# acoustic-warfare/beamforming-lk

Hardware: AMD Instinct MI355X
Metric: heatmap frames/sec (higher is better)
Workload: dtype f32

## Files before the change

### beamforming-lk_amd/_build.py

```python
from __future__ import annotations

import os
import shutil
import subprocess
from pathlib import Path

PKG_DIR = Path(__file__).resolve().parent
REPO = PKG_DIR.parent
CSRC = PKG_DIR / "csrc"
LIB_PATH = PKG_DIR / "libawpu_hip.so"

SOURCES = [CSRC / "das_kernels.hip", CSRC / "das_fast.hip", CSRC / "track_kernels.hip", CSRC / "block_kernels.hip", CSRC / "watch_kernels.hip", CSRC / "find_kernels.hip", CSRC / "band_kernels.hip", CSRC / "spectral_kernels.hip", CSRC / "expose_kernels.hip",
           CSRC / "awpu_hip.cpp", CSRC / "awpu_group.cpp", CSRC / "awpu_sweep.cpp", CSRC / "awpu_runs.cpp", CSRC / "geometry_host.cpp", CSRC / "find_host.cpp", CSRC / "band_host.cpp", CSRC / "spectral_host.cpp", CSRC / "awpu_focus.cpp", CSRC / "expose_host.cpp"]
GENERATOR = REPO / "tools" / "gen_trip_asm.py"
TRIP_INC = CSRC / "das_fast_trip.inc"
HEADERS = [CSRC / "awpu_handle.h", CSRC / "das_kernels.h", CSRC / "block_kernels.h", CSRC / "watch_kernels.h", CSRC / "find_kernels.h", CSRC / "find_rule.h", CSRC / "band_kernels.h", CSRC / "band_rule.h", CSRC / "spectral_kernels.h", CSRC / "spectral_rule.h", CSRC / "focus_rule.h", CSRC / "expose_kernels.h", CSRC / "expose_rule.h", CSRC / "nd_tile_window.h", CSRC / "sweep_plan.h", GENERATOR, REPO / "include" / "awpu_hip.h", REPO / "include" / "awpu_hip_track.h",
           REPO / "include" / "awpu_hip_blocks.h", REPO / "include" / "awpu_hip_listen.h", REPO / "include" / "awpu_hip_watch.h", REPO / "include" / "awpu_hip_find.h", REPO / "include" / "awpu_hip_band.h", REPO / "include" / "awpu_hip_focus.h", REPO / "include" / "awpu_hip_spectral.h", REPO / "include" / "awpu_hip_expose.h"]


def hipcc_path() -> str:
    for cand in (os.environ.get("HIPCC"), shutil.which("hipcc"), "/opt/rocm/bin/hipcc"):
        if cand and Path(cand).exists():
            return cand
    raise RuntimeError("hipcc not found: libawpu_hip.so cannot be built (there is no CPU fallback)")


def stale() -> bool:
    if not LIB_PATH.exists():
        return True
    built = LIB_PATH.stat().st_mtime
    return any(p.stat().st_mtime > built for p in SOURCES + HEADERS)


def build_library(force: bool = False, verbose: bool = False) -> Path:
    if not force and not stale():
        return LIB_PATH
    import fcntl

    with open(PKG_DIR / ".build.lock", "w") as lock:
        fcntl.flock(lock, fcntl.LOCK_EX)
        if not force and not stale():
            return LIB_PATH
        return _compile(verbose, force)


def generate_blocks(force: bool = False) -> Path:
    if not force and TRIP_INC.exists() and TRIP_INC.stat().st_mtime >= GENERATOR.stat().st_mtime:
        return TRIP_INC
    import sys
# ... 44 lines not shown
```

### beamforming-lk_amd/csrc/awpu_sweep.cpp

```cpp
#include "awpu_handle.h"

#include <algorithm>
#include <array>
#include <cstdio>
#include <cstdlib>
#include <cstring>
#include <map>
#include <vector>

#include "das_kernels.h"
#include "nd_tile_window.h"

using namespace awpu::host;

namespace {

int diag_begin(awpu_hip *h, size_t words, bool zero, hipStream_t s, unsigned long long **out) {
    if (const int rc = h->d_diag.ensure(words); rc != AWPU_OK) return rc;
    if (zero) AWPU_HIP_TRY(hipMemsetAsync(h->d_diag, 0, words * sizeof(unsigned long long), s));
    *out = h->d_diag;
    return AWPU_OK;
}

int diag_end(awpu_hip *h, int rc, size_t n_waves, int wg_waves, const char *tag, hipStream_t s) {
// ... 526 lines not shown
    a.n_pairs = (batch + 1) / 2;
    a.pair_group = awpu::xcd_pair_group((size_t) pp.usable_pad * pp.wr * 8, a.n_pairs);
    if (h->timing) AWPU_HIP_TRY(hipEventRecord(h->ev_begin, s));
    AWPU_HIP_TRY(awpu::launch_pack_pairs(d_frames, h->cfg.n_streams, hist_eff, wstart_eff, h->d_index, h->usable(), pp.usable_pad,
                                         h->d_gain, pp.wr, batch, h->d_pack, false, s));
    AWPU_HIP_TRY(awpu::launch_das_exact_quads(a, {table.entries, h->d_pack.cap}, s));
    return finish_launch(h, batch, s, AWPU_KERNEL_EXACT_QUAD);
}

int launch_exact_nd(awpu_hip *h, const float *d_frames, int batch, float *d_power, hipStream_t s, int hist_eff, int wstart_eff, int nq,
                    const float *prepacked = nullptr, size_t prepacked_floats = 0) {
    int rc = build_quad_lut(h, kQuadExactNd);
    if (rc != AWPU_OK) return rc;
    const QuadTable &table = h->quad_tables[kQuadExactNd];
    const awpu::FastPlan &pp = table.plan;
    if (!prepacked)
        if (const int prc = ensure_pack(h, pair_pack_floats(std::max(h->cfg.max_batch, batch), pp.usable_pad, pp.wr, 4)); prc != AWPU_OK) return prc;
    awpu::ExactNdArgs a{};
    fill_shared(a, h, pp, batch, d_power);
    a.packed = prepacked ? prepacked : h->d_pack;
    a.lut = table.d;
    a.sums = h->sums_out;
    a.wq = pp.wr;
    a.wq_tile = pp.row_bytes / 16;
    a.starts = h->d_nd_starts;
    a.start_entries = h->nd_start_entries;
    a.cols = h->cfg.grid_columns;
    a.rows = h->cfg.pixel_count / a.cols;
    a.nq = nq;
    a.tiles = awpu::nd_tiles(a.rows, a.cols, nq);
    a.n_pairs = (batch + 1) / 2;
    a.pair_group = awpu::xcd_pair_group((size_t) pp.usable_pad * pp.wr * 16, a.n_pairs, env().pair_group);
    if (env().pair_group <= 0 && a.pair_group == 2 && a.n_pairs >= 4 && (size_t) pp.usable_pad * pp.wr * 16 * 4 <= (6u << 20)) a.pair_group = 4;
    {
        const size_t items = (size_t) a.n_pairs * a.tiles;
        const long long key = ((long long) a.n_pairs << 24) | ((long long) a.pair_group << 8) | nq;
        if (!h->d_nd_items.holds(items)) {
            retire_live_graphs(h);
            AWPU_HIP_TRY(hipStreamSynchronize(s));
            if (rc = h->d_nd_items.grow(items); rc != AWPU_OK) return rc;
            h->nd_items_key = -1;
        }
        a.items = h->d_nd_items;
        a.build_items = h->nd_items_key != key;
        h->nd_items_key = key;
    }
    if (rc = arm_item_queues(h, a.n_pairs * a.tiles, &a.queue, &a.wgs, &a.tail); rc != AWPU_OK) return rc;
#ifdef AWPU_TUNING_BUILD
    if (const char *v = std::getenv("AWPU_ND_TAIL")) {
        const int per = (a.n_pairs * a.tiles + 7) / 8;
        a.tail = std::max(1, std::atoi(v) >= 100 ? per : per * std::atoi(v) / 100);
    }
#endif
    if (h->timing) AWPU_HIP_TRY(hipEventRecord(h->ev_begin, s));
    if (!prepacked) {
        AWPU_HIP_TRY(awpu::launch_pack_nd(d_frames, h->cfg.n_streams, hist_eff, wstart_eff, h->d_index, h->usable(), pp.usable_pad, h->d_gain,
                                          pp.wr, batch, h->d_pack, a.queue, s));
        a.queue_zeroed = 1;
    }
#ifdef AWPU_TUNING_BUILD
    const size_t n_wgs = std::min<size_t>((size_t) a.n_pairs * a.tiles, (size_t) a.wgs);
    if (env().debug & 16)
        if (const int drc = diag_begin(h, n_wgs * 8, true, s, &a.debug_out); drc != AWPU_OK) return drc;
#endif
    AWPU_HIP_TRY(awpu::launch_das_exact_nd(a, {table.entries, prepacked ? prepacked_floats : h->d_pack.cap}, s));
    rc = finish_launch(h, batch, s, AWPU_KERNEL_EXACT_ND);
#ifdef AWPU_TUNING_BUILD
    if (rc == AWPU_OK && (env().debug & 16)) return dump_nd_timeline(h, n_wgs, s);
#endif
    return rc;
}

bool takes_exact_nd(awpu_hip *h, int batch, int *nq) {
    if (!h->exact_pairs_ok || !h->exact_nd_ok || h->cfg.grid_columns < 1) return false;
    const ExactShape ex = env().exact_pairs;
    if (ex == ExactShape::kVerify || ex == ExactShape::kPair || ex == ExactShape::kQuad) return false;
    const int cols = h->cfg.grid_columns, rows = h->cfg.pixel_count / cols;
    const bool quads_pay = h->cfg.pixel_count % cols == 0 && h->cfg.pixel_begin % cols == 0 && h->quad_differ < 1.5;
    if ((!(h->pair_cols > 0 || quads_pay) && !forces_exact_nd(ex)) || rows < 4) return false;
    const long wgs2 = (long) awpu::nd_tiles(rows, cols, 2) * ((batch + 1) / 2);
    *nq = ex == ExactShape::kNd1 ? 1 : ex == ExactShape::kNd2 ? 2 : (rows >= 8 && wgs2 >= 512 ? 2 : 1);
    return true;
}

int arm_done_flag(awpu_hip *h, unsigned long long workgroups, awpu::DoneFlag *out) {
    if (!h->d_done_counter) {
        if (const int rc = h->d_done_counter.grow(1); rc != AWPU_OK) return rc;
        AWPU_HIP_TRY(hipMemsetAsync(h->d_done_counter, 0, sizeof(unsigned long long), h->stream));
        AWPU_HIP_TRY(hipStreamSynchronize(h->stream));
        if (const int rc = h->h_done_flag.grow(16); rc != AWPU_OK) return rc;
        *h->h_done_flag = 0;
        h->done_total = 0;
    }
    out->counter = h->d_done_counter;
    out->flag = h->h_done_flag;
    out->target = h->done_total + workgroups;
    out->seq = h->done_seq + 1;
    return AWPU_OK;
// ... 463 lines not shown
```

### beamforming-lk_amd/csrc/das_fast.hip

```cpp
#include "das_kernels.h"

#include <algorithm>
#include <atomic>

namespace awpu {

typedef float f2 __attribute__((ext_vector_type(2)));
typedef float f4 __attribute__((ext_vector_type(4)));
typedef float f4u __attribute__((ext_vector_type(4), aligned(4)));
typedef float f8 __attribute__((ext_vector_type(8)));

#define AWPU_AS4 __attribute__((address_space(4)))

typedef int i16 __attribute__((ext_vector_type(16)));

struct EntryGroup {
    i16 v;
    __device__ __forceinline__ float f(int k) const { return __int_as_float(v[4 * k + 0]); }
    __device__ __forceinline__ unsigned addr(int k) const { return (unsigned) v[4 * k + 1]; }
    __device__ __forceinline__ float g(int k) const { return __int_as_float(v[4 * k + 2]); }
};

template <int FPI>
struct Reads {
    f2 x[FPI], y[FPI];
};

__device__ __forceinline__ void no_fuse() { asm volatile("" ::: "memory"); }

template <int FPI>
__device__ __forceinline__ void issue_reads(Reads<FPI> &r, unsigned entry_addr, const char *lane_base) {
    constexpr int FS = kFastLdsBytes / FPI;
    const char *p = lane_base + entry_addr;
// ... 1072 lines not shown
    }
}

__device__ __forceinline__ f2 next_and_difference(float cur, float next, float gm) {
#pragma clang fp contract(off)
    const float c = cur * gm, n = next * gm;
    return f2{n, c - n};
}

__global__ void pack_nd_kernel(const float *frames, int n_streams, int hist, int wstart, const int32_t *index, int usable,
                               const float *gain, int wq, int batch, float *packed, unsigned *queue) {
    const int pair = blockIdx.y, s = blockIdx.x, rows_out = gridDim.x;
    if (queue && pair == 0 && s == 0 && threadIdx.x < 9) queue[threadIdx.x] = 0u;
    f4 *dst = (f4 *) packed + ((size_t) pair * rows_out + s) * wq;
    if (s >= usable) {
        for (int t = threadIdx.x; t < wq; t += blockDim.x) dst[t] = f4{0.0f, 0.0f, 0.0f, 0.0f};
        return;
    }
    const int fa = min(2 * pair, batch - 1), fb = min(2 * pair + 1, batch - 1);
    const float *xa = frames + ((size_t) fa * n_streams + index[s]) * hist + wstart;
    const float *xb = frames + ((size_t) fb * n_streams + index[s]) * hist + wstart;
    const float gm = gain ? gain[s] : 1.0f;
    const int valid = min(wq, hist - wstart - 1);
    for (int t = threadIdx.x; t < wq; t += blockDim.x) {
        f4 v = f4{0.0f, 0.0f, 0.0f, 0.0f};
        if (t < valid) {
            const f2 ea = next_and_difference(xa[t], xa[t + 1], gm), eb = next_and_difference(xb[t], xb[t + 1], gm);
            v = f4{ea.x, eb.x, ea.y, eb.y};
        }
        dst[t] = v;
    }
}

__global__ void nd_items_kernel(int2 *items, int n_pairs, int tiles, int pair_group, int tiles_per_row, int nq) {
    const int item = blockIdx.x * blockDim.x + threadIdx.x;
    if (item >= n_pairs * tiles) return;
    const int full_items = (n_pairs / pair_group) * pair_group * tiles;
    const int ga = item < full_items ? pair_group : n_pairs % pair_group;
    const int rem = item < full_items ? item : item - full_items;
    const int grp = rem / (tiles * ga), in = rem - grp * tiles * ga;
    const int tile = in / ga;
    const int pair = (item < full_items ? grp * pair_group : n_pairs - ga) + (in - tile * ga);
    const int rowq = tile / tiles_per_row, colt = tile - rowq * tiles_per_row;
    items[item] = int2{pair, (nq * rowq * tiles_per_row + colt) * 16};
}

struct NdQueues {
    unsigned *q;
    int per, total, tail;
    __device__ __forceinline__ int len(int x) const { return max(0, min(per, total - x * per)); }
    __device__ __forceinline__ int head(int x) const { return len(x) - min(len(x), tail); }
    __device__ __forceinline__ int take_head(int x) const {
        if (head(x) <= 0) return -1;
        const unsigned i = atomicAdd(&q[x], 1u);
        return i < (unsigned) head(x) ? x * per + (int) i : -1;
    }
    __device__ __forceinline__ int take_common() const {
        if (tail <= 0) return -1;
        for (;;) {
            const unsigned j = atomicAdd(&q[8], 1u);
            const int run = (int) (j / (unsigned) tail), k = (int) (j - (unsigned) run * (unsigned) tail);
            if (run >= 8) return -1;
            if (k < len(run) - head(run)) return run * per + head(run) + k;
        }
    }
    __device__ __forceinline__ int take(int xcd) const {
        int item = take_head(xcd);
        if (item < 0) item = take_common();
        for (int y = 1; item < 0 && y < 8; y++) item = take_head((xcd + y) & 7);
        return item;
    }
};

template <int NQ, bool SUMS>
__global__ __launch_bounds__(1024, 4) void das_exact_nd_kernel(ExactNdArgs a) {
    extern __shared__ __attribute__((aligned(16))) float lds[];
    constexpr int NW = 16, BUF = kFastLdsBytes;
    const int wave = __builtin_amdgcn_readfirstlane(threadIdx.x >> 6);
    const unsigned lds_base = (unsigned) (unsigned long long) (const __attribute__((address_space(3))) char *) lds;
    int *mail = (int *) (lds + 2 * (BUF / 4));
    const int total = a.n_pairs * a.tiles;
    unsigned xcc;
    asm volatile("s_getreg_b32 %0, hwreg(HW_REG_XCC_ID)" : "=s"(xcc));
    const NdQueues Q{a.queue, (total + 7) >> 3, total, a.tail};
    const int xcd = (int) (xcc & 7u);
    if (threadIdx.x == 0) {
        const int first = Q.take(xcd);
        mail[0] = first;
        mail[1] = first >= 0 ? Q.take(xcd) : -1;
    }
    __syncthreads();
    int cur = __builtin_amdgcn_readfirstlane(mail[0]), nxt = __builtin_amdgcn_readfirstlane(mail[1]);
    if (cur < 0) return;
    __syncthreads();

    const int tiles_per_row = (a.cols + NW - 1) / NW;
    auto decode = [&](int item, int &pair, int &tile_quad, const unsigned *&starts) {
        const int2 d = a.items[item];
        pair = __builtin_amdgcn_readfirstlane(d.x);
        tile_quad = __builtin_amdgcn_readfirstlane(d.y);
        const int quad_row = (tile_quad >> 4) / tiles_per_row, col_tile = (tile_quad >> 4) - quad_row * tiles_per_row;
        starts = a.starts + (size_t) ((quad_row >> 1) * tiles_per_row + col_tile) * a.usable_pad;
    };
    const int groups_total = a.usable_pad >> 2;
    const size_t row_floats = (size_t) a.wq * 4;
    const int n_chunks = (a.usable_pad + a.chunk - 1) / a.chunk;
    const int first_mics = min(a.chunk, a.usable_pad), last_mics = a.usable_pad - (n_chunks - 1) * a.chunk;
    const unsigned dbf = __builtin_amdgcn_readfirstlane((unsigned) ((size_t) a.chunk * row_floats * 4));
    const int row_bytes = a.wq_tile * 16;
    const int row_pieces = (row_bytes + 1023) >> 10;
    const unsigned last_shift = (unsigned) (row_pieces * 64 - a.wq_tile);
    const int rank = wave >> 2;
    const unsigned pka = __builtin_amdgcn_readfirstlane((unsigned) (first_mics >> 2) | (unsigned) (last_mics >> 2) << 8 | (unsigned) n_chunks << 16);
    const unsigned pkb_item = (wave < a.chunk ? (unsigned) row_pieces : 0u) | (wave < last_mics ? (unsigned) row_pieces : 0u) << 8 | last_shift << 24 |
                              (unsigned) rank << 30;
    const unsigned pkb_next = wave < first_mics ? (unsigned) row_pieces << 16 : 0u;
    const int own_head = Q.head(xcd);

    int pair, tile;
    const unsigned *starts;
    decode(cur, pair, tile, starts);
#ifdef AWPU_TUNING_BUILD
    const unsigned long long rt_begin = a.debug_out ? __builtin_amdgcn_s_memrealtime() : 0ull;
    long long t_sweep = 0, t_other = 0, t_mark = __builtin_readcyclecounter();
    int n_items = 0;
#endif
    {
        if (wave < first_mics) {
            const unsigned start = __builtin_amdgcn_readfirstlane(starts[wave]);
            const float *src = a.packed + ((size_t) pair * a.usable_pad + wave) * row_floats + (start >> 2);
            const int lane = (int) (threadIdx.x & 63);
            for (int k = 0; k < row_pieces; k++) {
                const int el = k * 64 + lane;
                if (el < a.wq_tile) {
                    float *dst = lds + ((wave * row_bytes) >> 2) + k * 256;
                    __builtin_amdgcn_global_load_lds((const __attribute__((address_space(1))) void *) (src + (size_t) el * 4),
                                                     (__attribute__((address_space(3))) void *) dst, 16, 0, 0);
                }
            }
        }
    }
    asm volatile("s_waitcnt vmcnt(0)" ::: "memory");
    __syncthreads();
    unsigned step = 0;

    for (;;) {
        const int cols_pad = tiles_per_row * NW;
        const int rowq = tile / (NQ * cols_pad);
        const int col = tile - NQ * rowq * cols_pad + wave;
        const int quad0 = tile + wave;
        const QuadEntry *quad_lut = a.lut + (size_t) quad0 * groups_total * 16;
        const float *pair_base = a.packed + (size_t) pair * a.usable_pad * row_floats;
        int pair_next = pair, tile_next = tile;
        const unsigned *starts_next = starts;
        if (nxt >= 0) decode(nxt, pair_next, tile_next, starts_next);
        const float *next_base = a.packed + (size_t) pair_next * a.usable_pad * row_floats;
        unsigned ticket = 0;
        const bool asked = wave == 0 && nxt >= 0 && own_head > 0;
        const unsigned *qptr = (const unsigned *) uniform_ptr(asked ? a.queue + xcd : nullptr);

        f8 O[NQ][4];
#ifdef AWPU_TUNING_BUILD
        { const long long n = __builtin_readcyclecounter(); t_other += n - t_mark; t_mark = n; }
#endif
        {
            unsigned tid = threadIdx.x;
            asm volatile("" : "+v"(tid));
            const unsigned lane_bytes = (tid & 63) * 16;
            const int buf = (int) (step & 1);
            unsigned lane_addr = lds_base + buf * BUF + lane_bytes;
            const unsigned ddst = __builtin_amdgcn_readfirstlane(lds_base + (buf ^ 1) * BUF + wave * row_bytes);
            const int delta = __builtin_amdgcn_readfirstlane(buf ? -BUF : BUF);
            const unsigned pkb = __builtin_amdgcn_readfirstlane(pkb_item | (nxt >= 0 ? pkb_next : 0u));
            const float *row_src = pair_base + (size_t) wave * row_floats, *row_next = next_base + (size_t) wave * row_floats;
            if constexpr (NQ == 1) {
                sweep_exact_nd_item1(O[0][0], O[0][1], O[0][2], O[0][3], uniform_ptr(quad_lut), pka, lane_addr, pkb, uniform_ptr(row_src), dbf,
                                     uniform_ptr(row_next), ddst, delta, lane_bytes, uniform_ptr(starts + wave), uniform_ptr(starts_next + wave), qptr, ticket);
            } else {
                static_assert(NQ == 2, "blocks are generated for one and two quads per wave");
                const int qstride = __builtin_amdgcn_readfirstlane(tiles_per_row * NW * groups_total * 16 * (int) sizeof(QuadEntry));
                sweep_exact_nd_item2(O[0][0], O[0][1], O[0][2], O[0][3], O[1][0], O[1][1], O[1][2], O[1][3], uniform_ptr(quad_lut), qstride, pka, lane_addr,
                                     pkb, uniform_ptr(row_src), dbf, uniform_ptr(row_next), ddst, delta, lane_bytes, uniform_ptr(starts + wave),
                                     uniform_ptr(starts_next + wave), qptr, ticket);
            }
            step += n_chunks;
        }
        if (threadIdx.x == 0 && nxt >= 0) {
            int got = own_head > 0 && ticket < (unsigned) own_head ? xcd * Q.per + (int) ticket : -1;
            if (got < 0) {
                got = Q.take_common();
                for (int y = 1; got < 0 && y < 8; y++) got = Q.take_head((xcd + y) & 7);
            }
            mail[0] = got;
        }
#ifdef AWPU_TUNING_BUILD
        { const long long n = __builtin_readcyclecounter(); t_sweep += n - t_mark; t_mark = n; n_items++; }
#endif

        unsigned tid_e = threadIdx.x;
        asm volatile("" : "+v"(tid_e));
        const int lane = (int) (tid_e & 63);
        const float norm = (float) (kSamples * a.usable);
#pragma unroll
        for (int q = 0; q < NQ; q++) {
            const int row4 = NQ * rowq + q;
            auto finish = [&](const f8 &Op, int pp) {
                const int row = 4 * row4 + pp;
                const bool live = row < a.rows && col < a.cols;
                const int p = min(row, a.rows - 1) * a.cols + min(col, a.cols - 1);
                f2 o[4];
#pragma unroll
                for (int k = 0; k < 4; k++) o[k] = f2{Op[2 * k], Op[2 * k + 1]};
                if (SUMS && live) {
#pragma unroll
                    for (int k = 0; k < 4; k++) {
                        a.sums[((size_t) (2 * pair) * a.pixel_count + p) * kSamples + lane + 64 * k] = o[k].x;
                        if (2 * pair + 1 < a.batch) a.sums[((size_t) (2 * pair + 1) * a.pixel_count + p) * kSamples + lane + 64 * k] = o[k].y;
                    }
                }
                return pixel_pair_partial_exact(o, lane);
            };
            const f2 s0 = finish(O[q][0], 0), s1 = finish(O[q][1], 1), s2 = finish(O[q][2], 2), s3 = finish(O[q][3], 3);
            const float sum = wave_sum8(s0.x, s0.y, s1.x, s1.y, s2.x, s2.y, s3.x, s3.y, lane);
            const int value = kWaveSum8Value(lane >> 3), row = 4 * row4 + (value >> 1), frame = 2 * pair + (value & 1);
            if ((lane & 7) == 0 && row < a.rows && col < a.cols && frame < a.batch)
                a.power[(size_t) frame * a.pixel_count + (size_t) row * a.cols + col] = sum / norm;
        }

        if (nxt < 0) break;
        __syncthreads();
        cur = nxt;
        pair = pair_next;
        tile = tile_next;
        starts = starts_next;
        nxt = __builtin_amdgcn_readfirstlane(mail[0]);
        __syncthreads();
    }
#ifdef AWPU_TUNING_BUILD
    if (a.debug_out && threadIdx.x == 0) {
        unsigned hw_id;
        asm volatile("s_getreg_b32 %0, hwreg(HW_REG_HW_ID)" : "=s"(hw_id));
        unsigned long long *o = a.debug_out + 8 * (size_t) blockIdx.x;
        o[0] = rt_begin;
        o[1] = __builtin_amdgcn_s_memrealtime();
        o[2] = (unsigned long long) t_other;
        o[3] = (unsigned long long) t_sweep;
        o[4] = (unsigned long long) (__builtin_readcyclecounter() - t_mark);
        o[5] = ((unsigned long long) xcc << 32) | hw_id;
        o[6] = (unsigned long long) n_items;
        o[7] = 1;
    }
#endif
}

__device__ __forceinline__ void store_tile_and_signal(float *lds, bool holder, int tile_row, int wave, int lane, float value, float *power, int row0,
                                                      int col0, int rows, int cols, const DoneFlag &done) {
    __syncthreads();
    if (holder) lds[tile_row * 16 + wave] = value;
    __syncthreads();
    if (wave != 0) return;
    const int r = row0 + (lane >> 4), c = col0 + (lane & 15);
    if (r < rows && c < cols) __hip_atomic_store(&power[(size_t) r * cols + c], lds[lane], __ATOMIC_RELAXED, __HIP_MEMORY_SCOPE_SYSTEM);
    asm volatile("s_waitcnt vmcnt(0)" ::: "memory");
    if (lane == 0 && __hip_atomic_fetch_add(done.counter, 1ull, __ATOMIC_RELAXED, __HIP_MEMORY_SCOPE_AGENT) + 1ull == done.target)
        __hip_atomic_store(done.flag, done.seq, __ATOMIC_RELAXED, __HIP_MEMORY_SCOPE_SYSTEM);
}

__global__ void pack_ndh_kernel(const float *frames, int n_streams, int pitch, int wstart, const int32_t *index, int usable,
// ... 349 lines not shown
        }
        sum.x = wave_sum(sum.x);
        sum.y = wave_sum(sum.y);
        const int p = pix[pp];
        if (lane == 0 && live[pp]) {
            a.power[(size_t) (2 * pair) * a.pixel_count + p] = sum.x / norm;
            if (2 * pair + 1 < a.batch) a.power[(size_t) (2 * pair + 1) * a.pixel_count + p] = sum.y / norm;
        }
    }
}

template <bool DIAG, int VAR>
__global__ __launch_bounds__(1024, 4) void das_quad_kernel(QuadArgs a) {
    extern __shared__ __attribute__((aligned(16))) float lds[];
    constexpr int NW = 16, kThreads = NW * 64, BUF = kFastLdsBytes;
    constexpr int kPieces = (BUF + kThreads * 16 - 1) / (kThreads * 16);
    const int lane = threadIdx.x & 63;
    const int wave = __builtin_amdgcn_readfirstlane(threadIdx.x >> 6);
    const unsigned lds_base = (unsigned) (unsigned long long) (const __attribute__((address_space(3))) char *) lds;

    const int total = a.n_pairs * a.tiles;
    const int per_xcd = (total + 7) >> 3;
    const int wgs_per_xcd = gridDim.x >> 3;
    const int run_begin = (blockIdx.x & 7) * per_xcd, run_end = min(total, run_begin + per_xcd);
    const int full_items = (a.n_pairs / a.pair_group) * a.pair_group * a.tiles;
    auto decode = [&](int item, int &pair, int &tile) {
        const int ga = item < full_items ? a.pair_group : a.n_pairs % a.pair_group;
        const int rem = item < full_items ? item : item - full_items;
        const int grp = rem / (a.tiles * ga), in = rem - grp * a.tiles * ga;
        tile = in / ga;
        pair = (item < full_items ? grp * a.pair_group : a.n_pairs - ga) + (in - tile * ga);
    };
    const bool queued = !DIAG && VAR == 0 && a.queue != nullptr;
    const NdQueues Q{a.queue, per_xcd, total, a.tail};
    int *mail = (int *) (lds + 2 * (BUF / 4));
    int xcd = (int) (blockIdx.x & 7);
    int item, nxt = -1;
    if (queued) {
        unsigned xcc;
        asm volatile("s_getreg_b32 %0, hwreg(HW_REG_XCC_ID)" : "=s"(xcc));
        xcd = (int) (xcc & 7u);
        if (threadIdx.x == 0) {
            const int first = Q.take(xcd);
            mail[0] = first;
            mail[1] = first >= 0 ? Q.take(xcd) : -1;
        }
        __syncthreads();
        item = __builtin_amdgcn_readfirstlane(mail[0]);
        nxt = __builtin_amdgcn_readfirstlane(mail[1]);
        if (item < 0) return;
        __syncthreads();
    } else {
        item = run_begin + (blockIdx.x >> 3);
        if (item >= run_end) return;
    }

    const int tiles_per_row4 = (a.cols + NW - 1) / NW;
    const int groups_total = a.usable_pad >> 2;
    const size_t row_floats = (size_t) a.wp * 2;
    const int n_chunks = (a.usable + a.chunk - 1) / a.chunk;
    const int rank = wave >> 2;
    const float norm = (float) (kSamples * a.usable);
    const int out_value = kWaveSum8Value(lane >> 3), out_pp = out_value >> 1, out_frame = out_value & 1;
    auto chunk_mics = [&](int m0) { return (min(a.chunk, a.usable - m0) + 3) & ~3; };
    const unsigned lane_bytes = threadIdx.x * 16;
    auto dma_chunk = [&](const float *src, int mc4, int buf) {
        const unsigned n_bytes = (unsigned) ((size_t) mc4 * row_floats * 4);
#pragma unroll
        for (int k = 0; k < kPieces; k++) {
            if (lane_bytes + k * kThreads * 16 < n_bytes) {
                const char *base = (const char *) uniform_ptr((const char *) src + k * kThreads * 16);
                float *dst = lds + buf * (BUF / 4) + (wave * 64 + k * kThreads) * 4;
                __builtin_amdgcn_global_load_lds((const __attribute__((address_space(1))) void *) (base + lane_bytes),
                                                 (__attribute__((address_space(3))) void *) dst, 16, 0, 0);
            }
        }
    };

// ... 19 lines not shown
    for (;;) {
        const int row4 = tile / tiles_per_row4;
        const int col = (tile - row4 * tiles_per_row4) * NW + wave;
        const int quad = row4 * tiles_per_row4 * NW + col;
        const QuadEntry *quad_lut = a.lut + (size_t) quad * groups_total * 16;
        const float *pair_base = a.packed + (size_t) pair * a.usable_pad * row_floats;
        const int item_next = queued ? nxt : item + wgs_per_xcd;
        const bool more = queued ? nxt >= 0 : item_next < run_end;
        int pair_next = 0, tile_next = 0;
        if (more) decode(item_next, pair_next, tile_next);

        f8 A0 = {0, 0, 0, 0, 0, 0, 0, 0}, A1 = A0, A2 = A0, A3 = A0, T = A0, V0 = A0, V2 = A0, V3 = A0;
        if constexpr (!DIAG && VAR == 0) {
            const int buf = step & 1;
            unsigned lane_addr = lds_base + buf * BUF + lane * 8;
            const int ngf = __builtin_amdgcn_readfirstlane(chunk_mics(0) >> 2);
            const int ngl = __builtin_amdgcn_readfirstlane(chunk_mics((n_chunks - 1) * a.chunk) >> 2);
            const unsigned dbf = __builtin_amdgcn_readfirstlane((unsigned) ((size_t) a.chunk * row_floats * 4));
            const unsigned dbl = __builtin_amdgcn_readfirstlane((unsigned) ((size_t) ngl * 4 * row_floats * 4));
            const float *nsrc = more ? a.packed + (size_t) pair_next * a.usable_pad * row_floats : pair_base;
            const unsigned dbn = __builtin_amdgcn_readfirstlane(more ? (unsigned) ((size_t) chunk_mics(0) * row_floats * 4) : 0u);
            const unsigned ddst = __builtin_amdgcn_readfirstlane(lds_base + (buf ^ 1) * BUF + wave * 1024);
            const int delta = __builtin_amdgcn_readfirstlane(buf ? -BUF : BUF);
            unsigned ticket = 0;
            const bool asked = queued && wave == 0 && more && Q.head(xcd) > 0;
            const unsigned *qptr = (const unsigned *) uniform_ptr(asked ? a.queue + xcd : nullptr);
            sweep_quad_item(A0, A1, A2, A3, T, V0, V2, V3, uniform_ptr(quad_lut), ngf, ngl, __builtin_amdgcn_readfirstlane(n_chunks),
                            lane_addr, rank, uniform_ptr(pair_base), dbf, dbl, uniform_ptr(nsrc), dbn, ddst, delta, lane_bytes, qptr, ticket);
            step += n_chunks;
            if (queued && threadIdx.x == 0 && more) {
                int got = Q.head(xcd) > 0 && ticket < (unsigned) Q.head(xcd) ? xcd * Q.per + (int) ticket : -1;
                if (got < 0) {
                    got = Q.take_common();
                    for (int y = 1; got < 0 && y < 8; y++) got = Q.take_head((xcd + y) & 7);
                }
                mail[0] = got;
            }
        } else
        for (int c = 0; c < n_chunks; c++, step++) {
            const int m0 = c * a.chunk;
            const int mc4 = chunk_mics(m0);
            const int buf = step & 1;
            long long t = DIAG ? __builtin_readcyclecounter() : 0;
            const int ng = __builtin_amdgcn_readfirstlane(mc4 >> 2);
            const int g_head = (a.debug & 512) ? __builtin_amdgcn_readfirstlane((ng * rank) >> 2) : 0;
            const unsigned lane_addr = lds_base + buf * BUF + lane * 8;
            auto sweep = [&](int g0, int n) {
                const void *row = uniform_ptr(quad_lut + (size_t) ((m0 >> 2) + g0) * 16);
                if constexpr (DIAG) {
                    unsigned dw = 0, da = 0;
                    sweep_quad_sum_stamped(A0, A1, A2, A3, T, V0, V2, V3, row, n, lane_addr, rank, dw, da);
                    t_wait += dw;
                    t_all += da;
                    n_blocks++;
                } else {
#ifdef AWPU_QUAD_VARIANTS
                    if constexpr (VAR == 1) sweep_quad_sum_v0(A0, A1, A2, A3, T, V0, V2, V3, row, n, lane_addr, rank);
                    else if constexpr (VAR == 2) sweep_quad_sum_v3(A0, A1, A2, A3, T, V0, V2, V3, row, n, lane_addr, rank);
                    else if constexpr (VAR == 3) sweep_quad_sum_v4(A0, A1, A2, A3, T, V0, V2, V3, row, n, lane_addr, rank);
                    else
#endif
                    sweep_quad_sum(A0, A1, A2, A3, T, V0, V2, V3, row, n, lane_addr, rank);
                }
            };
            const float *next_src = nullptr;
            int next_mc4 = 0;
            if (c + 1 < n_chunks) {
// ... 425 lines not shown
    if (a.cols > 0 && (unsigned) a.wp * 2u != kFirStaticPlaneBytes) return hipErrorInvalidValue;
    if ((a.wp & 3) || a.pair_group < 1 ||
        !within({(size_t) a.pixel_count * a.usable_pad + kFir8PlaneTablePrefetch, (size_t) n_pairs * a.usable * a.wp * 2}, have))
        return hipErrorInvalidValue;
    return launch_lds<das_fir8_plane_kernel<VAR>>(xcd_grid((long) n_pairs * n_tiles), dim3(1024), kTwoImages, stream, a,
                                                  (const FirPlaneEntry *) d_entries, d_coeffs, n_tiles, a.pair_group);
}

hipError_t launch_das_fir8_planes(const PairArgs &a, const void *d_entries, const float *d_coeffs, int variant, const Extents &have,
                                  hipStream_t stream) {
#ifdef AWPU_QUAD_VARIANTS
    if (variant == 1) return launch_fir8_plane_variant<1>(a, d_entries, d_coeffs, have, stream);
    if (variant == 2) return launch_fir8_plane_variant<2>(a, d_entries, d_coeffs, have, stream);
    if (variant == 3) return launch_fir8_plane_variant<3>(a, d_entries, d_coeffs, have, stream);
#endif
    (void) variant;
    return launch_fir8_plane_variant<0>(a, d_entries, d_coeffs, have, stream);
}

hipError_t launch_pack_nd(const float *d_frames, int n_streams, int hist, int wstart, const int32_t *d_index, int usable, int rows_out,
                          const float *d_gain, int wq, int batch, float *d_packed, unsigned *d_queue, hipStream_t stream) {
    hipLaunchKernelGGL(pack_nd_kernel, dim3(rows_out, (batch + 1) / 2), dim3(128), 0, stream, d_frames, n_streams, hist, wstart, d_index,
                       usable, d_gain, wq, batch, d_packed, d_queue);
    return hipGetLastError();
}

template <int NQ, bool SUMS>
static hipError_t launch_exact_nd_variant(const ExactNdArgs &a, hipStream_t stream) {
    const long total = (long) a.n_pairs * a.tiles;
    if (!a.queue_zeroed)
        if (hipError_t e = hipMemsetAsync(a.queue, 0, 9 * sizeof(unsigned), stream); e != hipSuccess) return e;
    if (a.build_items)
        hipLaunchKernelGGL(nd_items_kernel, dim3((unsigned) ((total + 255) / 256)), dim3(256), 0, stream, const_cast<int2 *>(a.items), a.n_pairs,
                           a.tiles, a.pair_group, (a.cols + 15) / 16, NQ);
    return launch_lds<das_exact_nd_kernel<NQ, SUMS>>(dim3((unsigned) std::min<long>(total, std::max(1, a.wgs))), dim3(1024),
                                                     kTwoImages + 64, stream, a);
}

hipError_t launch_das_exact_nd(const ExactNdArgs &a, const Extents &have, hipStream_t stream) {
    if ((a.nq != 1 && a.nq != 2) || !a.queue || !a.items || a.wgs < 1 || a.tail < 1) return hipErrorInvalidValue;
    if (!chunk_fits(a.chunk, a.usable_pad, (size_t) a.wq_tile * 16) || a.chunk > 16 || a.usable < 1 || a.usable > a.usable_pad || a.wq_tile < kSamples ||
        a.wq_tile > a.wq || !grid_is(a.rows, a.cols, a.pixel_count))
        return hipErrorInvalidValue;
    if (!items_agree(a.n_pairs, a.batch, a.tiles, nd_tiles(a.rows, a.cols, a.nq), a.pair_group)) return hipErrorInvalidValue;
    if (!a.starts || a.start_entries < (size_t) nd_tiles(a.rows, a.cols, 2) * a.usable_pad + 16) return hipErrorInvalidValue;
    if (!within({(size_t) nd_quad_count(a.rows, a.cols, a.nq) * (a.usable_pad / 4) * 16 + kQuadTablePrefetch,
                 (size_t) a.n_pairs * a.usable_pad * a.wq * 4}, have))
        return hipErrorInvalidValue;
    if (a.sums) return a.nq == 2 ? launch_exact_nd_variant<2, true>(a, stream) : launch_exact_nd_variant<1, true>(a, stream);
    return a.nq == 2 ? launch_exact_nd_variant<2, false>(a, stream) : launch_exact_nd_variant<1, false>(a, stream);
}

hipError_t launch_pack_ndh(const float *d_frames, int n_streams, int pitch, int wstart, const int32_t *d_index, int usable, int rows_out,
                           const float *d_gain, int wh, int batch, float *d_packed, hipStream_t stream) {
    hipLaunchKernelGGL(pack_ndh_kernel, dim3(rows_out, batch), dim3(256), 0, stream, d_frames, n_streams, pitch, wstart, d_index, usable, d_gain,
                       wh, d_packed);
    return hipGetLastError();
}

static bool ndh_shape_ok(const ExactNdhArgs &a, int tiles_of_grid, size_t image_bytes) {
    return chunk_fits(a.chunk, a.usable_pad, (size_t) a.wh * 16, image_bytes) && a.usable >= 1 && a.usable <= a.usable_pad && a.wh >= kSamples / 2 &&
           grid_is(a.rows, a.cols, a.pixel_count) && a.batch >= 1 && a.tiles == tiles_of_grid && (long) a.batch * a.tiles <= 0x7fffffffL;
}

template <int NQ, bool STATIONARY>
static hipError_t launch_exact_ndh_variant(const ExactNdhArgs &a, hipStream_t stream) {
    return launch_lds<das_exact_ndh_kernel<NQ, STATIONARY>>(dim3((unsigned) ((long) a.batch * a.tiles)), dim3(1024), kTwoImages, stream, a);
}

hipError_t launch_das_exact_ndh(const ExactNdhArgs &a, bool stationary, const Extents &have, hipStream_t stream) {
    if (a.nq != 1 && a.nq != 2) return hipErrorInvalidValue;
    if (!ndh_shape_ok(a, ndh_tiles(a.rows, a.cols, a.nq), stationary ? kTwoImages : kFastLdsBytes)) return hipErrorInvalidValue;
    if (stationary ? (a.chunk != a.usable_pad || !a.frames || !a.index || a.pitch < 1) : !a.packed) return hipErrorInvalidValue;
// ... 149 lines not shown
```

### beamforming-lk_amd/csrc/das_kernels.h

```cpp
#pragma once

#include <hip/hip_runtime.h>
#include <stdint.h>

#if defined(AWPU_TIMING_BUILD) && !defined(AWPU_TUNING_BUILD)
#define AWPU_TUNING_BUILD 1
#endif
#include "sweep_plan.h"

namespace awpu {

constexpr int kDebugNoRefill = 1, kDebugNoSweep = 2, kDebugNoTail = 4, kDebugNoBarrier = 8, kDebugRegStaging = 64;
constexpr int kDebugSafeBits = 16 | 256 | 512 | 4096;
#ifdef AWPU_TIMING_BUILD
#define AWPU_DBG(a, bit) ((a).debug & (bit))
#else
#define AWPU_DBG(a, bit) 0
#endif

struct LutEntry {
    int32_t off_rel;
    float frac;
};

// ... 68 lines not shown
    float *power;
    float *sums;
    int32_t usable, usable_pad, pixel_count, wp, chunk, batch;
    int32_t cols;
    int32_t tiles, n_pairs, pair_group;
};
hipError_t launch_das_exact_pairs(const ExactPairArgs &a, const Extents &have, hipStream_t stream);
struct ExactQuadArgs {
    const float *packed;
    const struct QuadEntry *lut;
    float *power;
    float *sums;
    int32_t usable, usable_pad, pixel_count, wp, chunk, batch;
    int32_t cols, rows;
    int32_t tiles, n_pairs, pair_group;
};
hipError_t launch_das_exact_quads(const ExactQuadArgs &a, const Extents &have, hipStream_t stream);
struct ExactNdArgs {
    const float *packed;
    const struct QuadEntry *lut;
    const unsigned *starts;
    size_t start_entries;
    int32_t wq_tile;
    float *power;
    float *sums;
    int32_t usable, usable_pad, pixel_count, wq, chunk, batch;
    int32_t cols, rows;
    int32_t nq;
    int32_t tiles, n_pairs, pair_group;
    unsigned *queue;
    int32_t queue_zeroed;
    int32_t wgs;
    int32_t tail;
    const int2 *items;
    int32_t build_items;
    unsigned long long *debug_out;
};
inline int nd_tiles(int rows, int cols, int nq) { return (((rows + 3) / 4 + nq - 1) / nq) * ((cols + 15) / 16); }
inline int nd_quad_count(int rows, int cols, int nq) { return (((rows + 3) / 4 + nq - 1) / nq) * nq * ((cols + 15) / 16) * 16; }
hipError_t launch_pack_nd(const float *d_frames, int n_streams, int hist, int wstart, const int32_t *d_index, int usable, int rows_out,
                          const float *d_gain, int wq, int batch, float *d_packed, unsigned *d_queue, hipStream_t stream);
hipError_t launch_das_exact_nd(const ExactNdArgs &a, const Extents &have, hipStream_t stream);
struct DoneFlag {
    unsigned long long *counter;
    unsigned *flag;
    unsigned long long target;
    uint32_t seq;
};
struct ExactNdhArgs {
    const float *packed;
    const float *frames;
    const struct QuadEntry *lut;
    const int32_t *index;
    const float *gain;
    float *power;
    float *sums;
    int32_t n_streams, pitch, wstart;
    int32_t usable, usable_pad, pixel_count, wh, chunk, batch;
    int32_t cols, rows;
    int32_t nq;
    int32_t tiles;
    int32_t lut_cols;
    int32_t identity;
    DoneFlag done;
};
inline int ndh_tiles(int rows, int cols, int nq) { return ((rows + 3) / 4) * ((cols + 16 * nq - 1) / (16 * nq)); }
// ... 210 lines not shown
```

Measured before the change: 24150.

## Claim runs of consecutive work items per queue ticket in exact ND kernel

Adds run-based work claiming to the exact ND kernel's per-XCD queues, so one atomic ticket can hand a workgroup up to four consecutive items. It also adds a tile_block ordering option to the item-list builder. The item descriptors for a run are prefetched through scalar loads, and the per-item block barriers and mailbox traffic are skipped inside a run. Both knobs default to 1 and can only be changed through environment variables in tuning builds, so the default path behaves like single-item claiming with some extra control flow.

```diff
diff --git a/beamforming-lk_amd/_build.py b/beamforming-lk_amd/_build.py
--- a/beamforming-lk_amd/_build.py
+++ b/beamforming-lk_amd/_build.py
@@ -14,7 +14,7 @@
            CSRC / "awpu_hip.cpp", CSRC / "awpu_group.cpp", CSRC / "awpu_sweep.cpp", CSRC / "awpu_runs.cpp", CSRC / "geometry_host.cpp", CSRC / "find_host.cpp", CSRC / "band_host.cpp", CSRC / "spectral_host.cpp", CSRC / "awpu_focus.cpp", CSRC / "expose_host.cpp"]
 GENERATOR = REPO / "tools" / "gen_trip_asm.py"
 TRIP_INC = CSRC / "das_fast_trip.inc"
-HEADERS = [CSRC / "awpu_handle.h", CSRC / "das_kernels.h", CSRC / "block_kernels.h", CSRC / "watch_kernels.h", CSRC / "find_kernels.h", CSRC / "find_rule.h", CSRC / "band_kernels.h", CSRC / "band_rule.h", CSRC / "spectral_kernels.h", CSRC / "spectral_rule.h", CSRC / "focus_rule.h", CSRC / "expose_kernels.h", CSRC / "expose_rule.h", CSRC / "nd_tile_window.h", CSRC / "sweep_plan.h", GENERATOR, REPO / "include" / "awpu_hip.h", REPO / "include" / "awpu_hip_track.h",
+HEADERS = [CSRC / "awpu_handle.h", CSRC / "das_kernels.h", CSRC / "block_kernels.h", CSRC / "watch_kernels.h", CSRC / "find_kernels.h", CSRC / "find_rule.h", CSRC / "band_kernels.h", CSRC / "band_rule.h", CSRC / "spectral_kernels.h", CSRC / "spectral_rule.h", CSRC / "focus_rule.h", CSRC / "expose_kernels.h", CSRC / "expose_rule.h", CSRC / "nd_queue_rule.h", CSRC / "nd_tile_window.h", CSRC / "sweep_plan.h", GENERATOR, REPO / "include" / "awpu_hip.h", REPO / "include" / "awpu_hip_track.h",
            REPO / "include" / "awpu_hip_blocks.h", REPO / "include" / "awpu_hip_listen.h", REPO / "include" / "awpu_hip_watch.h", REPO / "include" / "awpu_hip_find.h", REPO / "include" / "awpu_hip_band.h", REPO / "include" / "awpu_hip_focus.h", REPO / "include" / "awpu_hip_spectral.h", REPO / "include" / "awpu_hip_expose.h"]
 
 
diff --git a/beamforming-lk_amd/csrc/awpu_sweep.cpp b/beamforming-lk_amd/csrc/awpu_sweep.cpp
--- a/beamforming-lk_amd/csrc/awpu_sweep.cpp
+++ b/beamforming-lk_amd/csrc/awpu_sweep.cpp
@@ -582,9 +582,13 @@
     a.n_pairs = (batch + 1) / 2;
     a.pair_group = awpu::xcd_pair_group((size_t) pp.usable_pad * pp.wr * 16, a.n_pairs, env().pair_group);
     if (env().pair_group <= 0 && a.pair_group == 2 && a.n_pairs >= 4 && (size_t) pp.usable_pad * pp.wr * 16 * 4 <= (6u << 20)) a.pair_group = 4;
+    a.tile_block = 1;
+#ifdef AWPU_TUNING_BUILD
+    if (const char *v = std::getenv("AWPU_ND_TILE_BLOCK")) a.tile_block = std::clamp(std::atoi(v), 1, 63);
+#endif
+    const long long items_key = ((long long) a.n_pairs << 24) | ((long long) a.pair_group << 8) | ((long long) a.tile_block << 2) | nq;
     {
         const size_t items = (size_t) a.n_pairs * a.tiles;
-        const long long key = ((long long) a.n_pairs << 24) | ((long long) a.pair_group << 8) | nq;
         if (!h->d_nd_items.holds(items)) {
             retire_live_graphs(h);
             AWPU_HIP_TRY(hipStreamSynchronize(s));
@@ -592,8 +596,7 @@
             h->nd_items_key = -1;
         }
         a.items = h->d_nd_items;
-        a.build_items = h->nd_items_key != key;
-        h->nd_items_key = key;
+        a.build_items = h->nd_items_key != items_key;
     }
     if (rc = arm_item_queues(h, a.n_pairs * a.tiles, &a.queue, &a.wgs, &a.tail); rc != AWPU_OK) return rc;
 #ifdef AWPU_TUNING_BUILD
@@ -601,6 +604,10 @@
         const int per = (a.n_pairs * a.tiles + 7) / 8;
         a.tail = std::max(1, std::atoi(v) >= 100 ? per : per * std::atoi(v) / 100);
     }
+#endif
+    a.run = 1;
+#ifdef AWPU_TUNING_BUILD
+    if (const char *v = std::getenv("AWPU_ND_RUN")) a.run = std::clamp(std::atoi(v), 1, 4);
 #endif
     if (h->timing) AWPU_HIP_TRY(hipEventRecord(h->ev_begin, s));
     if (!prepacked) {
@@ -613,7 +620,9 @@
     if (env().debug & 16)
         if (const int drc = diag_begin(h, n_wgs * 8, true, s, &a.debug_out); drc != AWPU_OK) return drc;
 #endif
+    if (a.build_items) h->nd_items_key = -1;
     AWPU_HIP_TRY(awpu::launch_das_exact_nd(a, {table.entries, prepacked ? prepacked_floats : h->d_pack.cap}, s));
+    h->nd_items_key = items_key;
     rc = finish_launch(h, batch, s, AWPU_KERNEL_EXACT_ND);
 #ifdef AWPU_TUNING_BUILD
     if (rc == AWPU_OK && (env().debug & 16)) return dump_nd_timeline(h, n_wgs, s);
diff --git a/beamforming-lk_amd/csrc/das_fast.hip b/beamforming-lk_amd/csrc/das_fast.hip
--- a/beamforming-lk_amd/csrc/das_fast.hip
+++ b/beamforming-lk_amd/csrc/das_fast.hip
@@ -1,4 +1,5 @@
 #include "das_kernels.h"
+#include "nd_queue_rule.h"
 
 #include <algorithm>
 #include <atomic>
@@ -1137,45 +1138,22 @@
     }
 }
 
-__global__ void nd_items_kernel(int2 *items, int n_pairs, int tiles, int pair_group, int tiles_per_row, int nq) {
+__global__ void nd_items_kernel(int2 *items, int n_pairs, int tiles, int pair_group, int tiles_per_row, int nq, int tile_block) {
     const int item = blockIdx.x * blockDim.x + threadIdx.x;
     if (item >= n_pairs * tiles) return;
     const int full_items = (n_pairs / pair_group) * pair_group * tiles;
     const int ga = item < full_items ? pair_group : n_pairs % pair_group;
     const int rem = item < full_items ? item : item - full_items;
     const int grp = rem / (tiles * ga), in = rem - grp * tiles * ga;
-    const int tile = in / ga;
-    const int pair = (item < full_items ? grp * pair_group : n_pairs - ga) + (in - tile * ga);
+    const int blk = in / (tile_block * ga), in_blk = in - blk * tile_block * ga;
+    const int blk_tiles = min(tile_block, tiles - blk * tile_block);
+    const int pair_in = in_blk / blk_tiles;
+    const int tile = blk * tile_block + (in_blk - pair_in * blk_tiles);
+    const int pair = (item < full_items ? grp * pair_group : n_pairs - ga) + pair_in;
     const int rowq = tile / tiles_per_row, colt = tile - rowq * tiles_per_row;
     items[item] = int2{pair, (nq * rowq * tiles_per_row + colt) * 16};
 }
 
-struct NdQueues {
-    unsigned *q;
-    int per, total, tail;
-    __device__ __forceinline__ int len(int x) const { return max(0, min(per, total - x * per)); }
-    __device__ __forceinline__ int head(int x) const { return len(x) - min(len(x), tail); }
-    __device__ __forceinline__ int take_head(int x) const {
-        if (head(x) <= 0) return -1;
-        const unsigned i = atomicAdd(&q[x], 1u);
-        return i < (unsigned) head(x) ? x * per + (int) i : -1;
-    }
-    __device__ __forceinline__ int take_common() const {
-        if (tail <= 0) return -1;
-        for (;;) {
-            const unsigned j = atomicAdd(&q[8], 1u);
-            const int run = (int) (j / (unsigned) tail), k = (int) (j - (unsigned) run * (unsigned) tail);
-            if (run >= 8) return -1;
-            if (k < len(run) - head(run)) return run * per + head(run) + k;
-        }
-    }
-    __device__ __forceinline__ int take(int xcd) const {
-        int item = take_head(xcd);
-        if (item < 0) item = take_common();
-        for (int y = 1; item < 0 && y < 8; y++) item = take_head((xcd + y) & 7);
-        return item;
-    }
-};
 
 template <int NQ, bool SUMS>
 __global__ __launch_bounds__(1024, 4) void das_exact_nd_kernel(ExactNdArgs a) {
@@ -1187,21 +1165,37 @@
     const int total = a.n_pairs * a.tiles;
     unsigned xcc;
     asm volatile("s_getreg_b32 %0, hwreg(HW_REG_XCC_ID)" : "=s"(xcc));
-    const NdQueues Q{a.queue, (total + 7) >> 3, total, a.tail};
+    const NdQueues Q{a.queue, (total + 7) >> 3, total, a.tail, a.run};
     const int xcd = (int) (xcc & 7u);
     if (threadIdx.x == 0) {
-        const int first = Q.take(xcd);
-        mail[0] = first;
-        mail[1] = first >= 0 ? Q.take(xcd) : -1;
+        const NdRun first = Q.take(xcd);
+        const NdRun second = first.first >= 0 ? Q.take(xcd) : NdRun{-1, 0};
+        mail[0] = first.first;
+        mail[1] = first.len;
+        mail[2] = second.first;
+        mail[3] = second.len;
     }
     __syncthreads();
-    int cur = __builtin_amdgcn_readfirstlane(mail[0]), nxt = __builtin_amdgcn_readfirstlane(mail[1]);
+    const int cur = __builtin_amdgcn_readfirstlane(mail[0]);
+    int left = __builtin_amdgcn_readfirstlane(mail[1]) - 1;
+    int run_next = __builtin_amdgcn_readfirstlane(mail[2]), len_next = __builtin_amdgcn_readfirstlane(mail[3]);
     if (cur < 0) return;
     __syncthreads();
 
     const int tiles_per_row = (a.cols + NW - 1) / NW;
-    auto decode = [&](int item, int &pair, int &tile_quad, const unsigned *&starts) {
-        const int2 d = a.items[item];
+    typedef const __attribute__((address_space(4))) int *ItemList;
+    auto adopt = [&](int first, int len, int2 &d0, int2 &d1, int2 &d2, int2 &d3) {
+        const ItemList it = (ItemList) (unsigned long long) uniform_ptr(a.items + first);
+        d0 = int2{it[0], it[1]};
+        d1 = d2 = d3 = d0;
+        if (len > 1) {
+            const int i1 = 2, i2 = 2 * min(2, len - 1), i3 = 2 * min(3, len - 1);
+            d1 = int2{it[i1], it[i1 + 1]};
+            d2 = int2{it[i2], it[i2 + 1]};
+            d3 = int2{it[i3], it[i3 + 1]};
+        }
+    };
+    auto decode = [&](int2 d, int &pair, int &tile_quad, const unsigned *&starts) {
         pair = __builtin_amdgcn_readfirstlane(d.x);
         tile_quad = __builtin_amdgcn_readfirstlane(d.y);
         const int quad_row = (tile_quad >> 4) / tiles_per_row, col_tile = (tile_quad >> 4) - quad_row * tiles_per_row;
@@ -1224,7 +1218,12 @@
 
     int pair, tile;
     const unsigned *starts;
-    decode(cur, pair, tile, starts);
+    int2 after0, after1, after2;
+    {
+        int2 d0;
+        adopt(cur, left + 1, d0, after0, after1, after2);
+        decode(d0, pair, tile, starts);
+    }
 #ifdef AWPU_TUNING_BUILD
     const unsigned long long rt_begin = a.debug_out ? __builtin_amdgcn_s_memrealtime() : 0ull;
     long long t_sweep = 0, t_other = 0, t_mark = __builtin_readcyclecounter();
@@ -1256,12 +1255,23 @@
         const int quad0 = tile + wave;
         const QuadEntry *quad_lut = a.lut + (size_t) quad0 * groups_total * 16;
         const float *pair_base = a.packed + (size_t) pair * a.usable_pad * row_floats;
+        const bool run_ends = left == 0;
+        const bool more = !run_ends || run_next >= 0;
+        const bool switches = run_ends && run_next >= 0;
         int pair_next = pair, tile_next = tile;
         const unsigned *starts_next = starts;
-        if (nxt >= 0) decode(nxt, pair_next, tile_next, starts_next);
+        if (switches) {
+            int2 d0;
+            adopt(run_next, len_next, d0, after0, after1, after2);
+            decode(d0, pair_next, tile_next, starts_next);
+        } else if (!run_ends) {
+            decode(after0, pair_next, tile_next, starts_next);
+            after0 = after1;
+            after1 = after2;
+        }
         const float *next_base = a.packed + (size_t) pair_next * a.usable_pad * row_floats;
         unsigned ticket = 0;
-        const bool asked = wave == 0 && nxt >= 0 && own_head > 0;
+        const bool asked = wave == 0 && switches && own_head > 0;
         const unsigned *qptr = (const unsigned *) uniform_ptr(asked ? a.queue + xcd : nullptr);
 
         f8 O[NQ][4];
@@ -1276,7 +1286,7 @@
             unsigned lane_addr = lds_base + buf * BUF + lane_bytes;
             const unsigned ddst = __builtin_amdgcn_readfirstlane(lds_base + (buf ^ 1) * BUF + wave * row_bytes);
             const int delta = __builtin_amdgcn_readfirstlane(buf ? -BUF : BUF);
-            const unsigned pkb = __builtin_amdgcn_readfirstlane(pkb_item | (nxt >= 0 ? pkb_next : 0u));
+            const unsigned pkb = __builtin_amdgcn_readfirstlane(pkb_item | (more ? pkb_next : 0u));
             const float *row_src = pair_base + (size_t) wave * row_floats, *row_next = next_base + (size_t) wave * row_floats;
             if constexpr (NQ == 1) {
                 sweep_exact_nd_item1(O[0][0], O[0][1], O[0][2], O[0][3], uniform_ptr(quad_lut), pka, lane_addr, pkb, uniform_ptr(row_src), dbf,
@@ -1290,13 +1300,11 @@
             }
             step += n_chunks;
         }
-        if (threadIdx.x == 0 && nxt >= 0) {
-            int got = own_head > 0 && ticket < (unsigned) own_head ? xcd * Q.per + (int) ticket : -1;
-            if (got < 0) {
-                got = Q.take_common();
-                for (int y = 1; got < 0 && y < 8; y++) got = Q.take_head((xcd + y) & 7);
-            }
-            mail[0] = got;
+        if (threadIdx.x == 0 && switches) {
+            NdRun got = Q.head_run(xcd, ticket);
+            if (got.first < 0) got = Q.take_elsewhere(xcd);
+            mail[0] = got.first;
+            mail[1] = got.len;
         }
 #ifdef AWPU_TUNING_BUILD
         { const long long n = __builtin_readcyclecounter(); t_sweep += n - t_mark; t_mark = n; n_items++; }
@@ -1332,13 +1340,18 @@
                 a.power[(size_t) frame * a.pixel_count + (size_t) row * a.cols + col] = sum / norm;
         }
 
-        if (nxt < 0) break;
-        __syncthreads();
-        cur = nxt;
+        if (!more) break;
         pair = pair_next;
         tile = tile_next;
         starts = starts_next;
-        nxt = __builtin_amdgcn_readfirstlane(mail[0]);
+        if (!run_ends) {
+            left--;
+            continue;
+        }
+        __syncthreads();
+        left = len_next - 1;
+        run_next = __builtin_amdgcn_readfirstlane(mail[0]);
+        len_next = __builtin_amdgcn_readfirstlane(mail[1]);
         __syncthreads();
     }
 #ifdef AWPU_TUNING_BUILD
@@ -1754,7 +1767,7 @@
         pair = (item < full_items ? grp * a.pair_group : a.n_pairs - ga) + (in - tile * ga);
     };
     const bool queued = !DIAG && VAR == 0 && a.queue != nullptr;
-    const NdQueues Q{a.queue, per_xcd, total, a.tail};
+    const NdQueues Q{a.queue, per_xcd, total, a.tail, 1};
     int *mail = (int *) (lds + 2 * (BUF / 4));
     int xcd = (int) (blockIdx.x & 7);
     int item, nxt = -1;
@@ -1763,9 +1776,9 @@
         asm volatile("s_getreg_b32 %0, hwreg(HW_REG_XCC_ID)" : "=s"(xcc));
         xcd = (int) (xcc & 7u);
         if (threadIdx.x == 0) {
-            const int first = Q.take(xcd);
+            const int first = Q.take_item(xcd);
             mail[0] = first;
-            mail[1] = first >= 0 ? Q.take(xcd) : -1;
+            mail[1] = first >= 0 ? Q.take_item(xcd) : -1;
         }
         __syncthreads();
         item = __builtin_amdgcn_readfirstlane(mail[0]);
@@ -1851,7 +1864,7 @@
                 int got = Q.head(xcd) > 0 && ticket < (unsigned) Q.head(xcd) ? xcd * Q.per + (int) ticket : -1;
                 if (got < 0) {
                     got = Q.take_common();
-                    for (int y = 1; got < 0 && y < 8; y++) got = Q.take_head((xcd + y) & 7);
+                    for (int y = 1; got < 0 && y < 8; y++) got = Q.take_head_item((xcd + y) & 7);
                 }
                 mail[0] = got;
             }
@@ -2343,13 +2356,13 @@
         if (hipError_t e = hipMemsetAsync(a.queue, 0, 9 * sizeof(unsigned), stream); e != hipSuccess) return e;
     if (a.build_items)
         hipLaunchKernelGGL(nd_items_kernel, dim3((unsigned) ((total + 255) / 256)), dim3(256), 0, stream, const_cast<int2 *>(a.items), a.n_pairs,
-                           a.tiles, a.pair_group, (a.cols + 15) / 16, NQ);
+                           a.tiles, a.pair_group, (a.cols + 15) / 16, NQ, a.tile_block);
     return launch_lds<das_exact_nd_kernel<NQ, SUMS>>(dim3((unsigned) std::min<long>(total, std::max(1, a.wgs))), dim3(1024),
                                                      kTwoImages + 64, stream, a);
 }
 
 hipError_t launch_das_exact_nd(const ExactNdArgs &a, const Extents &have, hipStream_t stream) {
-    if ((a.nq != 1 && a.nq != 2) || !a.queue || !a.items || a.wgs < 1 || a.tail < 1) return hipErrorInvalidValue;
+    if ((a.nq != 1 && a.nq != 2) || !a.queue || !a.items || a.wgs < 1 || a.tail < 1 || a.run < 1 || a.run > 4 || a.tile_block < 1) return hipErrorInvalidValue;
     if (!chunk_fits(a.chunk, a.usable_pad, (size_t) a.wq_tile * 16) || a.chunk > 16 || a.usable < 1 || a.usable > a.usable_pad || a.wq_tile < kSamples ||
         a.wq_tile > a.wq || !grid_is(a.rows, a.cols, a.pixel_count))
         return hipErrorInvalidValue;
diff --git a/beamforming-lk_amd/csrc/das_kernels.h b/beamforming-lk_amd/csrc/das_kernels.h
--- a/beamforming-lk_amd/csrc/das_kernels.h
+++ b/beamforming-lk_amd/csrc/das_kernels.h
@@ -124,6 +124,8 @@
     int32_t queue_zeroed;
     int32_t wgs;
     int32_t tail;
+    int32_t run;
+    int32_t tile_block;
     const int2 *items;
     int32_t build_items;
     unsigned long long *debug_out;
diff --git a/beamforming-lk_amd/csrc/nd_queue_rule.h b/beamforming-lk_amd/csrc/nd_queue_rule.h
--- /dev/null
+++ b/beamforming-lk_amd/csrc/nd_queue_rule.h
@@ -0,0 +1,76 @@
+#pragma once
+
+#if defined(__HIPCC__) || defined(__CUDACC__)
+#define AWPU_QUEUE_FN __host__ __device__ __forceinline__
+#else
+#define AWPU_QUEUE_FN inline
+#endif
+
+namespace awpu {
+
+struct NdRun {
+    int first, len;
+};
+
+struct NdQueues {
+    unsigned *q;
+    int per, total, tail;
+    int run;
+
+    static AWPU_QUEUE_FN unsigned add_one(unsigned *counter) {
+#if defined(__HIP_DEVICE_COMPILE__) || defined(__CUDA_ARCH__)
+        return atomicAdd(counter, 1u);
+#else
+        return (*counter)++;
+#endif
+    }
+    static AWPU_QUEUE_FN int lo(int a, int b) { return a < b ? a : b; }
+    AWPU_QUEUE_FN int len(int x) const {
+        const int n = lo(per, total - x * per);
+        return n > 0 ? n : 0;
+    }
+    AWPU_QUEUE_FN int head(int x) const { return len(x) - lo(len(x), tail); }
+    AWPU_QUEUE_FN NdRun head_run(int x, unsigned r) const {
+        const int h = head(x);
+        if (h <= 0 || r >= (unsigned) h) return NdRun{-1, 0};
+        const unsigned at = r * (unsigned) run;
+        if (at >= (unsigned) h) return NdRun{-1, 0};
+        return NdRun{x * per + (int) at, lo(run, h - (int) at)};
+    }
+    AWPU_QUEUE_FN NdRun take_head(int x) const {
+        if (head(x) <= 0) return NdRun{-1, 0};
+        return head_run(x, add_one(&q[x]));
+    }
+    AWPU_QUEUE_FN int take_common() const {
+        if (tail <= 0) return -1;
+        for (;;) {
+            const unsigned j = add_one(&q[8]);
+            const int share = (int) (j / (unsigned) tail), k = (int) (j - (unsigned) share * (unsigned) tail);
+            if (share >= 8) return -1;
+            if (k < len(share) - head(share)) return share * per + head(share) + k;
+        }
+    }
+    AWPU_QUEUE_FN NdRun take_elsewhere(int xcd) const {
+        const int item = take_common();
+        NdRun got{item, item >= 0 ? 1 : 0};
+        for (int y = 1; got.first < 0 && y < 8; y++) got = take_head((xcd + y) & 7);
+        return got;
+    }
+    AWPU_QUEUE_FN int take_head_item(int x) const {
+        if (head(x) <= 0) return -1;
+        const unsigned i = add_one(&q[x]);
+        return i < (unsigned) head(x) ? x * per + (int) i : -1;
+    }
+    AWPU_QUEUE_FN int take_item(int xcd) const {
+        int item = take_head_item(xcd);
+        if (item < 0) item = take_common();
+        for (int y = 1; item < 0 && y < 8; y++) item = take_head_item((xcd + y) & 7);
+        return item;
+    }
+    AWPU_QUEUE_FN NdRun take(int xcd) const {
+        const NdRun got = take_head(xcd);
+        return got.first >= 0 ? got : take_elsewhere(xcd);
+    }
+};
+
+}
```

After: 24180, median of 5. Within noise of the previous version (+0.1%).
